# shunpeizhang/nebula

Measured on AMD Instinct MI355X. Metric: GO 3 STEPS traversed edges/sec (TEPS) at 1/2/4/8 GPU; FIND SHORTEST PATH p50, higher is better.
Workload: dtype int64; 1 GPU; GO 3 STEPS FROM <root> OVER e WHERE e.w < 50 YIELD e._dst, 16 single-root queries per step; graph=RMAT-26, parts=100, roots=16, queries_in_flight=6, parallelism=single, vertices_rank0=32799492, live_edges_out_plus_in_rank0=2120776948

## Files before the change

### nebula_amd/csrc/kernels.hip

```cpp
#include <hip/hip_runtime.h>
#include <array>
#include <cstddef>

#include <cstdio>
#include <cstring>
#include <vector>

#include "aggops.h"
#include "stage.h"
#include "ws.h"

namespace nbg {


struct DegSrc {
  const uint32_t* row_ptr;
  const uint8_t* visible;
  uint32_t cap;
};

struct ListOut {
  uint32_t* ids;
  uint32_t* seg_end;
  uint32_t* seg_rs;
// ... 2607 lines not shown
    launch(dim3(mark_grid(il->n, il->total)), 0, w->stream, a, nullptr, w->seg_end, w->seg_rs, w->flags, FinalParams{},
           bp, &w->q->e_st[step][tix], &w->q->step_n[step], il);
    prof_end(w, p, K_EXPAND_MARK, step, tix);
    return hipGetLastError();
  }
  const ListRef L = prepare_list(w, a0, n_bound, step, tix);
  ExpandArgs a = a0;
  a.frontier = L.ids;
  a.tsplit = set_split(w, L.set);
  FinalParams fp{};
  fp.err_flag = &w->q->err;
  hipEvent_t p = prof_begin(w, K_EXPAND_MARK);
  launch(dim3(mark_grid(n_bound, e_bound)), 0, w->stream, a, L.acc, set_end(w, L.set), set_rs(w, L.set), w->flags, fp,
         bp, &w->q->e_st[step][tix], L.stat_n, nullptr);
  prof_end(w, p, K_EXPAND_MARK, step, tix);
  return hipGetLastError();
}

void ws_set_wake(Workspace* w, bool flag) { w->wake_flag = flag; }

void ws_set_mark_claims(Workspace* w, bool claims) {
  const bool flags = w->env_flags || !claims;
  if (flags != w->mark_flags) (void)hipMemsetAsync(&w->q->acc[2], 0, 3 * sizeof(unsigned long long), w->stream);
  w->mark_flags = flags;
}

hipError_t ws_finish_step(Workspace* w, int step, const ExpandArgs* next0) {
  if (w->mark_flags) return ws_compact(w, step, next0);
  w->cur ^= 1;
  w->list_acc = &w->q->acc[2 + (step + 1) % 3];
  w->seg_ready = next0 != nullptr;
  return hipSuccess;
}

hipError_t ws_compact(Workspace* w, int step, const ExpandArgs* next0) {
  unsigned long long* acc = &w->q->acc[2 + w->pc];
  unsigned long long* other = &w->q->acc[2 + (w->pc ^ 1)];
  w->pc ^= 1;
  uint32_t* next = w->frontier[w->cur ^ 1];
  hipEvent_t p = prof_begin(w, K_COMPACT);
  hipLaunchKernelGGL(k_compact, dim3((unsigned)(w->flag_bytes / CP_BYTES)), dim3(CP_THREADS), 0, w->stream, w->flags,
                     deg_src(next0), list_out(w, next, acc, other, nullptr, w->cur ^ 1));
  prof_end(w, p, K_COMPACT, step, 0);
  w->cur ^= 1;
  w->list_acc = acc;
  w->seg_ready = next0 != nullptr;
  return hipGetLastError();
}

static int edge_columns_read(const TypeProgram& prog) {
  uint64_t seen = 0;
  int n = 0;
  for (auto& ins : prog.code) {
    if (ins.op != OP_COL && ins.op != OP_COLV) continue;
    const uint64_t bit = 1ull << (ins.aux & 63);
    if (!(seen & bit)) { seen |= bit; ++n; }
  }
  return n;
}

static const void* col_ptr(const ExpandArgs& a, int c, int* bytes) {
  if (a.hnarrow && a.hnarrow[c]) {
    *bytes = a.hnarrow_bytes[c];
    return a.hnarrow[c];
  }
  *bytes = 8;
  return a.hprops[c];
}

static FastProg detect_fast(const TypeProgram& prog, const ExpandArgs& a) {
  FastProg f{};
  f.enabled = 0;
  auto leaf_col = [&](const Ins& i) {
    return (i.op == OP_COL || (i.op == OP_COLV && a.valid == nullptr)) && a.hprops != nullptr;
  };
  if (prog.where_reg >= 0) {
    if (prog.where_len != 3) return f;
    const Ins &i0 = prog.code[0], &i1 = prog.code[1], &c = prog.code[2];
    static const int kOps[6] = {OP_LT_I, OP_LE_I, OP_GT_I, OP_GE_I, OP_EQ_I, OP_NE_I};
    static const int kSwap[6] = {2, 3, 0, 1, 4, 5};
    int op = -1;
    for (int k = 0; k < 6; ++k)
      if (c.op == kOps[k]) op = k;
    if (op < 0 || c.d != prog.where_reg) return f;
    const Ins* colI = nullptr;
    const Ins* constI = nullptr;
    if (leaf_col(i0) && i1.op == OP_CONST) { colI = &i0; constI = &i1; }
    else if (i0.op == OP_CONST && leaf_col(i1)) { colI = &i1; constI = &i0; }
    else return f;
    if (c.a == colI->d && c.b == constI->d) {
    } else if (c.a == constI->d && c.b == colI->d) {
      op = kSwap[op];
    } else {
      return f;
    }
    const int64_t k = constI->imm;
    f.lo = INT64_MIN;
    f.hi = INT64_MAX;
    switch (op) {
      case 0: if (k == INT64_MIN) { f.lo = 1; f.hi = 0; } else f.hi = k - 1; break;
      case 1: f.hi = k; break;
      case 2: if (k == INT64_MAX) { f.lo = 1; f.hi = 0; } else f.lo = k + 1; break;
      case 3: f.lo = k; break;
      case 4: f.lo = f.hi = k; break;
      default: f.lo = f.hi = k; f.where_neg = 1; break;
    }
    f.has_where = 1;
    f.wcol = col_ptr(a, colI->aux, &f.wbytes);
  }
  const int ny = (int)prog.yield_reg.size();
  int pc = prog.where_len;
  for (int y = 0; y < ny; ++y) {
    if (prog.yield_reg[y] < 0) { f.ykind[y] = 4; continue; }
    if (pc >= (int)prog.code.size()) return f;
    const Ins& i = prog.code[pc++];
    if (i.d != prog.yield_reg[y]) return f;
    if (i.op == OP_DST) { f.ykind[y] = 0; f.dst_yield = 1; }
    else if (i.op == OP_SRC) f.ykind[y] = 1;
    else if (i.op == OP_RANK) f.ykind[y] = 2;
    else if (i.op == OP_EIDX) f.ykind[y] = 5;
    else if (leaf_col(i)) { f.ykind[y] = 3; f.ycol[y] = col_ptr(a, i.aux, &f.ybytes[y]); }
    else return f;
  }
  if (pc != (int)prog.code.size()) return f;
  f.enabled = 1;
  return f;
}

static unsigned final_grid(uint64_t n_bound, uint64_t e_bound) {
  const char* ev = getenv("NBG_FINAL_GRID");
  const unsigned cap = ev ? (unsigned)atoi(ev) : 0u;
  const unsigned g = expand_grid(n_bound, e_bound);
  return cap && cap < g ? cap : g;
}

unsigned ws_final_grid(uint64_t n_bound, uint64_t e_bound) { return final_grid(n_bound, e_bound); }

uint64_t ws_final_blk_cap(uint64_t n_bound, uint64_t e_bound) {
  const uint64_t tiles = cdiv(n_bound + e_bound + 1, TILE);
  const uint64_t waves = (uint64_t)final_grid(n_bound, e_bound) * WAVES;
  return cdiv(tiles, waves) * WAVES * TILE;
}

uint64_t ws_shard_cap(uint64_t n_bound, uint64_t e_bound) {
  uint64_t tiles = cdiv(n_bound + e_bound + 1, TILE);
  return cdiv(tiles, NSHARD) * TILE;
}

static bool lean_final() {
  static const bool on = !getenv("NBG_FINAL_LEAN") || atoi(getenv("NBG_FINAL_LEAN")) != 0;
  return on;
}

static bool final_where_shape(const FastProg& f, const ExpandArgs& a) {
  bool dst_only = f.enabled != 0;
  for (int y = 0; y < MAX_YIELDS; ++y) dst_only = dst_only && (f.ykind[y] == 0 || f.ykind[y] == 4);
  return dst_only && lean_final() && f.dst_yield && a.dst_vid && f.has_where && f.wcol;
}

bool ws_final_where(const TypeProgram& prog, const ExpandArgs& a, StmtIndexSpec* sp) {
  if (prog.yield_reg.size() > (size_t)MAX_YIELDS) return false;
  const FastProg f = detect_fast(prog, a);
  if (!final_where_shape(f, a)) return false;
  sp->row_ptr = a.row_ptr;
  sp->dst_vid = a.dst_vid;
  sp->wcol = f.wcol;
  sp->wbytes = f.wbytes;
  sp->lo = f.lo;
  sp->hi = f.hi;
  sp->where_neg = f.where_neg;
  return true;
}

hipError_t ws_expand_final(Workspace* w, const ExpandArgs& a0, uint64_t n_bound, uint64_t e_bound, int step, int tix,
                           const TypeProgram& prog, uint64_t region_base, uint64_t blk_cap, const InlineList* il,
                           const uint32_t* full_row_ptr) {
  if (step > MAX_STEPS || tix >= MAX_TYPES_Q) return hipErrorInvalidValue;
  const bool inl = inline_start_list(w, tix, il);
  if (full_row_ptr && (inl || tix != 0 || !w->seg_ready)) return hipErrorInvalidValue;
  const ListRef L = inl ? ListRef{nullptr, nullptr, &w->q->step_n[step], 0} : prepare_list(w, a0, n_bound, step, tix);
  ExpandArgs a = a0;
  a.frontier = L.ids;
  a.tsplit = inl ? nullptr : set_split(w, L.set);
  uint32_t* const l_end = set_end(w, L.set);
  uint32_t* const l_rs = set_rs(w, L.set);
  FinalParams fp{};
  fp.prog = w->d_prog + (size_t)tix * MAX_PROGRAM;
  fp.where_len = prog.where_len;
  fp.where_reg = prog.where_reg;
  fp.prog_len = (int)prog.code.size();
  fp.nyields = (int)prog.yield_reg.size();
  for (int y = 0; y < fp.nyields; ++y) {
    fp.yield_reg[y] = prog.yield_reg[y];
    fp.yield_const[y] = prog.yield_const[y];
  }
  for (int y = 0; y < MAX_YIELDS; ++y) fp.out_cols[y] = ws_row_col(w, y < w->ncols_alloc ? y : 0);
  fp.region_base = region_base;
  fp.blk_cap = blk_cap;
  fp.blk_rows = w->blk_rows + (size_t)tix * EXPAND_GRID;
  fp.err_flag = &w->q->err;
  fp.probe_mask = prog.probe_mask;
  fp.keep_on_error = prog.keep_on_error ? 1 : 0;
  fp.tag_bits = &w->q->tagbits;
  a.str.arena = w->sarena;
  a.str.arena_cap = w->sarena_cap;
  a.str.arena_used = &w->q->arena_used;
  a.str.err_flag = &w->q->err;
  fp.fast = detect_fast(prog, a);
  if (full_row_ptr) {
    if (!final_where_shape(fp.fast, a)) return hipErrorInvalidValue;
    fp.fast.has_where = 0;
    fp.fast.wcol = nullptr;
    fp.fast.wbytes = 0;
  }
  size_t lds = fp.fast.enabled ? 0 : (size_t)(prog.nregs > 0 ? prog.nregs : 1) * BLOCK * sizeof(int64_t);
  bool dst_only = fp.fast.enabled;
  for (int y = 0; y < fp.nyields; ++y) dst_only = dst_only && (fp.fast.ykind[y] == 0 || fp.fast.ykind[y] == 4);
  const bool wide = fp.fast.enabled && !dst_only && fp.nyields >= 4 && e_bound <= (1ull << 20);
  hipEvent_t p = prof_begin(w, K_EXPAND_FINAL);
  const dim3 grid(final_grid(n_bound, e_bound));
  unsigned long long* e_st = &w->q->e_st[step][tix];
  const auto launch = dst_only ? launch_expand<FINALD>
                      : wide ? launch_expand<FINALY>
                      : fp.fast.enabled ? launch_expand<FINALF> : launch_expand<FINAL>;
  if (!inl && dst_only && lean_final() && fp.fast.dst_yield && a.dst_vid && (!fp.fast.has_where || fp.fast.wcol)) {
    FinalDstArgs fa{};
    fa.acc = L.acc;
    fa.seg_end = l_end;
    fa.seg_rs = l_rs;
    fa.tsplit = a.tsplit;
    fa.tsplit_n = w->cap_tiles;
    fa.dst_vid = a.dst_vid;
    fa.wcol = fp.fast.wcol;
    fa.lo = fp.fast.lo;
    fa.hi = fp.fast.hi;
    fa.where_neg = fp.fast.where_neg;
    fa.nyields = fp.nyields;
    for (int y = 0; y < fp.nyields; ++y) {
      if (fp.fast.ykind[y] != 0) fa.const_mask |= 1ull << y;
      fa.yconst[y] = fp.yield_const[y];
      fa.out[y] = fp.out_cols[y];
    }
    fa.region_base = region_base;
    fa.blk_cap = blk_cap;
    fa.blk_rows = fp.blk_rows;
    fa.stat_e = e_st;
    if (full_row_ptr) {
      fa.full_rp = full_row_ptr;
      fa.ids = L.ids;
      fa.visible = a.visible;
    }
    fa.stat_n = L.stat_n;
    fa.err_flag = &w->q->err;
    const bool one = fp.nyields == 1 && fa.const_mask == 0;
    const hipError_t le = launch_final_dst(fa, fp.fast.has_where ? fp.fast.wbytes : 0, one, grid.x, w->stream);
    if (le != hipSuccess) {
      prof_end(w, p, K_EXPAND_FINAL, step, tix, 0.0, 0.0);
      return le;
    }
  } else {
    launch(grid, lds, w->stream, a, L.acc, l_end, l_rs, w->flags, fp, BfsParams{}, e_st, L.stat_n, inl ? il : nullptr);
  }
  prof_end(w, p, K_EXPAND_FINAL, step, tix, full_row_ptr ? -1.0 : (double)edge_columns_read(prog), (double)fp.nyields);
  w->final_grid[tix] = final_grid(n_bound, e_bound);
  return hipGetLastError();
}



hipError_t ws_backtracker(Workspace* w, int64_t** out, int64_t** in) {
  if (!w->bt) HIP_TRY(hipMalloc((void**)&w->bt, (w->nv + 1) * 8));
  if (w->comm && !w->h_btc) {
    const uint64_t G = (uint64_t)w->comm->world, nwords = G * w->npad / 64;
    if (!w->bt_out) HIP_TRY(hipMalloc((void**)&w->bt_out, G * w->npad * 8));
    if (!w->bt_pack) HIP_TRY(hipMalloc((void**)&w->bt_pack, G * w->npad * 8));
    if (!w->bt_recv) HIP_TRY(hipMalloc((void**)&w->bt_recv, G * w->npad * 8));
    if (!w->bt_pre) HIP_TRY(hipMalloc((void**)&w->bt_pre, 2 * nwords * 4));
    if (!w->bt_boff) HIP_TRY(hipMalloc((void**)&w->bt_boff, 2 * (nwords / RW_BLOCK) * 4));
    if (!w->bt_disp) HIP_TRY(hipMalloc((void**)&w->bt_disp, 2 * G * 8));
    HIP_TRY(hipHostMalloc((void**)&w->h_btc, 2 * G * 8, hipHostMallocMapped | hipHostMallocCoherent));
    HIP_TRY(hipHostGetDevicePointer((void**)&w->d_btc, w->h_btc, 0));
  }
  w->bt_active = true;
  *in = w->bt;
  *out = w->comm ? w->bt_out : w->bt;
  return hipSuccess;
}

void ws_backtracker_off(Workspace* w) { w->bt_active = false; }

hipError_t ws_scan_only(Workspace* w, const ExpandArgs& a, uint64_t n_bound, int step, int tix) {
  const ListRef L = prepare_list(w, a, n_bound, step, tix);
  hipLaunchKernelGGL(k_note, dim3(1), dim3(1), 0, w->stream, L.acc, &w->q->e_st[step][tix], L.stat_n);
  return hipGetLastError();
}




struct Wake {
  unsigned long long* word;
  unsigned int* ticket;
  unsigned long long seq;
};
__device__ void wake_host(const Wake& wk) {
  if (!wk.word) return;
  __builtin_amdgcn_fence(__ATOMIC_RELEASE, "");
  __syncthreads();
  if (threadIdx.x != 0) return;
  if (gridDim.x > 1) {
    const unsigned got = __hip_atomic_fetch_add(wk.ticket, 1u, __ATOMIC_RELEASE, __HIP_MEMORY_SCOPE_AGENT);
    if (got != gridDim.x - 1) return;
    __builtin_amdgcn_fence(__ATOMIC_ACQUIRE, "agent");
    __hip_atomic_store(wk.ticket, 0u, __ATOMIC_RELAXED, __HIP_MEMORY_SCOPE_AGENT);
  }
  __hip_atomic_store(wk.word, wk.seq, __ATOMIC_RELEASE, __HIP_MEMORY_SCOPE_SYSTEM);
}

__global__ void __launch_bounds__(BLOCK) k_q_out(unsigned long long* __restrict__ src, unsigned long long* dst,
                                                 uint32_t n8, uint32_t nq8, Wake wk) {
  for (uint32_t i = threadIdx.x; i < n8; i += BLOCK) {
    dst[i] = src[i];
    if (i < nq8) src[i] = 0;
  }
  wake_host(wk);
}

static bool wake_by_flag() {
  static const bool on = !(getenv("NBG_WAKE") && strcmp(getenv("NBG_WAKE"), "event") == 0) &&
                         getenv("NBG_BLOCKING_SYNC") == nullptr;
  return on;
}

static Wake arm_wake(Workspace* w) {
  w->wake_armed = wake_by_flag() && w->wake_flag && !w->comm;
  if (!w->wake_armed) return Wake{nullptr, nullptr, 0};
  return Wake{w->d_wake, w->d_ticket, ++w->wake_seq};
}

static hipError_t wait_wake(Workspace* w) {
  const unsigned long long want = w->wake_seq;
  for (unsigned k = 1;; ++k) {
    if (__atomic_load_n(w->h_wake, __ATOMIC_ACQUIRE) == want) {
      (void)hipEventQuery(w->done_ev);
      return hipSuccess;
    }
    if ((k & 255) == 0) {
      const hipError_t e = hipEventQuery(w->done_ev);
      if (e == hipErrorNotReady) continue;
      if (__atomic_load_n(w->h_wake, __ATOMIC_ACQUIRE) == want) return hipSuccess;
      return e == hipSuccess ? hipErrorLaunchFailure : e;
    }
  }
}

hipError_t ws_end_query_async(Workspace* w) {
  int nt = 0;
  for (int t = 0; t < MAX_TYPES_Q; ++t)
    if (w->final_grid[t]) nt = t + 1;
  static_assert(sizeof(QState) % 8 == 0 && EXPAND_GRID % 2 == 0, "k_q_out copies 8-byte words");
  const size_t bytes = sizeof(QState) + (size_t)nt * EXPAND_GRID * 4;
  const Wake wk = arm_wake(w);
  hipLaunchKernelGGL(k_q_out, dim3(1), dim3(BLOCK), 0, w->stream, reinterpret_cast<unsigned long long*>(w->q),
                     reinterpret_cast<unsigned long long*>(w->d_hq), (uint32_t)(bytes / 8),
                     (uint32_t)(sizeof(QState) / 8), wk);
  w->q_reset = true;
  HIP_TRY(hipGetLastError());
  if (w->h_small) w->h_small[0] = 0;
  if (!w->done_ev) HIP_TRY(hipEventCreateWithFlags(&w->done_ev, hipEventDisableTiming));
  return hipEventRecord(w->done_ev, w->stream);
}

hipError_t ws_end_query_wait(Workspace* w) {
  static const bool blocking = getenv("NBG_BLOCKING_SYNC") != nullptr;
  if (w->comm) {
    HIP_TRY(ws_sync(w));
  } else if (w->wake_armed) {
    w->wake_armed = false;
    HIP_TRY(wait_wake(w));
  } else if (blocking) {
    HIP_TRY(hipEventSynchronize(w->done_ev));
  } else {
    hipError_t e;
    while ((e = hipEventQuery(w->done_ev)) == hipErrorNotReady) {
    }
    HIP_TRY(e);
  }
  if (!w->q_reset) HIP_TRY(hipMemsetAsync(w->q, 0, sizeof(QState), w->stream));
  w->q_reset = false;
  prof_flush(w, w->h_q);
  return hipSuccess;
}

constexpr int SMALL_SEGS = 2048;
constexpr int SMALL_WGS = 16;
__global__ void __launch_bounds__(BLOCK) k_q_out_small(unsigned long long* __restrict__ src, unsigned long long* dst,
                                                       uint32_t n8, uint32_t nq8, const uint32_t* __restrict__ blk_rows, SmallPack sp,
                                                       int64_t* const* __restrict__ cols, int64_t* small, Wake wk) {
  for (uint32_t i = blockIdx.x * BLOCK + threadIdx.x; i < n8; i += gridDim.x * BLOCK) {
    dst[i] = src[i];
    if (i < nq8) src[i] = 0;
  }
  __shared__ uint32_t s_seg[SMALL_SEGS];
  __shared__ uint32_t s_off[SMALL_SEGS + 1];
  __shared__ uint32_t s_lds[WAVES];
  __shared__ uint32_t s_n, s_rows;
  if (threadIdx.x == 0) s_n = s_rows = 0;
  __syncthreads();
// ... 1453 lines not shown
```

### nebula_amd/csrc/nbg_internal.h

```cpp
#pragma once
#include <hip/hip_runtime_api.h>

#include <array>
#include <cstdint>
#include <map>
#include <memory>
#include <string>
#include <unordered_map>
#include <vector>

#include "../../include/nbg.h"

namespace nbg {

constexpr uint32_t NO_ROW = 0xFFFFFFFFu;

struct Column {
  std::string name;
  int32_t type;
};
struct Schema {
  int64_t version = 0;
  std::vector<Column> cols;
  int find(const std::string& n) const {
// ... 166 lines not shown
constexpr uint64_t STR_HASH_MASK = ((uint64_t)1 << 62) - 1;
inline bool is_derived_code(int64_t c) { return ((uint64_t)c >> 62) == 1; }
constexpr int64_t STR_INPUT = (int64_t)1 << 61;
constexpr int64_t STR_ARENA = (int64_t)1 << 60;
inline bool is_input_code(int64_t c) { return ((uint64_t)c >> 61) == 1; }
constexpr uint64_t STR_HASH_INIT = 0xcbf29ce484222325ull;

#if defined(__HIPCC__)
#define NBG_HD __host__ __device__
#else
#define NBG_HD
#endif
NBG_HD inline uint64_t str_hash_step(uint64_t h, uint8_t b) { return (h ^ b) * 0x100000001b3ull; }
NBG_HD inline int64_t str_derived_code(uint64_t h, uint64_t len) {
  uint64_t z = h ^ (len * 0x9E3779B97F4A7C15ull);
  z = (z ^ (z >> 30)) * 0xBF58476D1CE4E5B9ull;
  z = (z ^ (z >> 27)) * 0x94D049BB133111EBull;
  z ^= z >> 31;
  return STR_DERIVED | (int64_t)(z & STR_HASH_MASK);
}

struct DevStrings {
  const uint32_t* off = nullptr;
  const char* bytes = nullptr;
  const int64_t* s2i = nullptr;
  const int64_t* s2f = nullptr;
  const uint8_t* s2ok = nullptr;
  uint64_t n = 0;
  const uint32_t* xoff = nullptr;
  const char* xbytes = nullptr;
  uint64_t xn = 0;
  char* arena = nullptr;
  unsigned long long* arena_used = nullptr;
  uint64_t arena_cap = 0;
  unsigned long long* err_flag = nullptr;
};
constexpr unsigned long long ARENA_OVERFLOW = 1ull << 32;
constexpr unsigned long long SPLIT_BAD = 1ull << 48;

constexpr int MAX_REGS = 48;
int interp_max_regs();
int tiny_max_regs();
constexpr int MAX_PROGRAM = 256;
constexpr int MAX_YIELDS = 32;

struct TypeProgram {
  int32_t etype = 0;
  std::vector<Ins> code;
  int where_len = 0;
  int where_reg = -1;
  VKind where_kind = VK_BOOL;
  bool where_const = false;
  bool where_const_val = true;
  bool where_always_error = false;
  std::vector<int> yield_reg;
  std::vector<VKind> yield_kind;
  std::vector<int64_t> yield_const;
  std::vector<std::string> yield_const_str;
  std::vector<Ins> data;
  bool sout = false;
  uint64_t sout_bytes = 0;
  bool needs_error_check = false;
  uint32_t probe_mask = 0;
  bool keep_on_error = false;
  int nregs = 0;
};

#ifndef NBG_VT
#define NBG_VT 4
#endif
constexpr int VT = NBG_VT;
constexpr int TILE = 64 * VT;
constexpr int NSHARD = 64;
constexpr int MAX_STEPS = 32;
constexpr int MAX_TYPES_Q = 32;
constexpr int INLINE_STARTS = 32;
constexpr int MAX_TAG_BITS = 16;
constexpr int MAX_INPUT_COLS = 32;

struct InlineList {
  uint32_t n;
  uint32_t n_in;
  uint32_t total;
  uint32_t id[INLINE_STARTS];
  uint32_t end[INLINE_STARTS];
  uint32_t rs[INLINE_STARTS];
};

struct QState {
  unsigned long long n;
  unsigned long long total;
  unsigned long long err;
  unsigned long long acc[5];
  unsigned long long step_n[MAX_STEPS + 2];
  unsigned long long e_st[MAX_STEPS + 2][MAX_TYPES_Q];
  unsigned long long tagbits;
  unsigned long long arena_used;
};

struct ExpandArgs {
  const uint32_t* frontier;
  const uint32_t* row_ptr;
  const uint32_t* col;
  const int64_t* dst_vid;
  const int64_t* rank;
  const uint8_t* valid;
  const uint8_t* visible;
  const int64_t* vids;
  const int64_t* const* props;
  uint32_t cap;
  const uint32_t* tsplit;
  const int64_t* const* hprops;
  void* const* hnarrow;
  const int* hnarrow_bytes;
  const int64_t* const* tcols;
  const uint8_t* const* tpres;
  uint32_t gbase;
  int64_t* bt;
  const int64_t* bt_in;
  int bt_first;
  const int64_t* in_ids;
  uint64_t in_n;
  const int64_t* const* in_cols;
  DevStrings str;
  int64_t now_sec;
  uint64_t rand_seed;
};

struct FinalDstArgs {
  const unsigned long long* acc;
  const uint32_t* seg_end;
  const uint32_t* seg_rs;
  const uint32_t* tsplit;
  uint64_t tsplit_n;
  const int64_t* dst_vid;
  const void* wcol;
  int64_t lo, hi;
  int32_t where_neg;
  int32_t nyields;
  uint64_t const_mask;
  int64_t yconst[MAX_YIELDS];
  int64_t* out[MAX_YIELDS];
  uint64_t region_base, blk_cap;
  uint32_t* blk_rows;
  unsigned long long* stat_e;
  unsigned long long* stat_n;
  unsigned long long* err_flag;
  const uint32_t* full_rp;
  const uint32_t* ids;
  const uint8_t* visible;
};
hipError_t launch_final_dst(const FinalDstArgs& a, int wbytes, bool one, unsigned grid, hipStream_t s);

struct StmtIndexSpec {
  const uint32_t* row_ptr;
  const int64_t* dst_vid;
  uint64_t nv, edges;
  const void* wcol;
  int wbytes;
  int64_t lo, hi;
  int where_neg;
};
struct StmtIndex {
  uint32_t* rp = nullptr;
  int64_t* dst = nullptr;
  uint64_t rows = 0;
  uint64_t bytes = 0;
};
bool stmtidx_build(const StmtIndexSpec& sp, uint64_t budget_bytes, hipStream_t s, StmtIndex* out, double* ms);
void stmtidx_free(StmtIndex* ix);

constexpr int LVL_BITS = 6;
constexpr uint32_t MAX_PATH_LEN = (1u << LVL_BITS) - 1;
constexpr int PSLOTS = 8;
enum PathLabel { LAB_F = 0, LAB_B = 1, LAB_S = 2, LAB_M = 3, NUM_LABS = 4 };
constexpr int GREEDY_HOP_BLOCKS = 64;
constexpr int PATH_REC = 64;

struct PState {
  unsigned long long n[PSLOTS];
  unsigned long long total;
  unsigned long long edges;
  unsigned long long meets;
  unsigned long long found;
  unsigned long long err;
  unsigned long long acc[2];
  unsigned long long dsum[2];
  unsigned long long shard[NSHARD];
  unsigned long long ln[PATH_REC];
  unsigned long long le[PATH_REC];
  unsigned long long lc[PATH_REC];
  unsigned long long gticket;
  unsigned long long gv;
  unsigned long long gpart[4 * GREEDY_HOP_BLOCKS];
  unsigned long long ld[PATH_REC];
  unsigned long long mdsum;
  unsigned long long mdsum_out;
};

struct PathTypes {
  int n = 0;
  int32_t type[MAX_TYPES_Q];
  ExpandArgs a[MAX_TYPES_Q];
};

struct SpTypes {
  int n = 0;
  int32_t type[MAX_TYPES_Q];
  const uint32_t* row_ptr[MAX_TYPES_Q];
  const uint32_t* col[MAX_TYPES_Q];
  const int64_t* dst_vid[MAX_TYPES_Q];
  const int64_t* rank[MAX_TYPES_Q];
  uint64_t ne[MAX_TYPES_Q];
};
struct SpResult {
  unsigned long long L;
  unsigned long long edges;
  unsigned long long err;
  unsigned long long levels;
  unsigned long long abytes;
  unsigned long long launches;
  unsigned long long batches;
  long long path[1 + 3 * MAX_PATH_LEN];
};
constexpr unsigned long long CH_ERR_WALK_CAP = 64;
inline std::string sp_err_text(unsigned long long err) {
  if (err == CH_ERR_WALK_CAP) return "greedy walk incomplete at the chain's launch cap";
  if (err & 4) return "a frontier list's merge-path split did not describe its tile (code " + std::to_string(err) + ")";
  return "device search aborted (code " + std::to_string(err) + ")";
}
constexpr uint32_t CH_LAB_WORDS = 4;
struct SpCtx;
enum SpMode : int { SP_CHAIN = 1 };
SpCtx* sp_create(uint64_t nv, uint64_t item_cap, uint64_t edge_cap, hipStream_t s, std::string* err);
void sp_destroy(SpCtx* c);
hipError_t sp_launch(SpCtx* c, const SpTypes& fwd, const SpTypes& bwd, const uint8_t* visible, const int64_t* vids,
                     uint32_t s, uint32_t t, uint32_t upto, uint64_t dmin = 0);
bool sp_ready(SpCtx* c);
struct SpPair {
  const SpTypes* fwd;
  const SpTypes* bwd;
  const uint8_t* visible;
  const int64_t* vids;
  uint32_t s, t, upto;
};
hipError_t sp_launch_batch(SpCtx* const* cs, int n, const SpPair* pairs);
struct ChainCtx;
ChainCtx* chain_create(uint64_t nv, uint64_t edge_cap, hipStream_t s, std::string* err, uint64_t list_cap = 0);
void sp_set_list_cap(SpCtx* c, uint64_t list_cap);
void chain_destroy(ChainCtx* c);
hipError_t chain_launch(ChainCtx* c, const SpTypes& fwd, const SpTypes& bwd, const uint8_t* visible,
                        const int64_t* vids, uint32_t* const lab[3], uint32_t epoch, uint32_t s, uint32_t t,
                        uint32_t upto, uint64_t dmin = 0);
bool chain_more(ChainCtx* c, hipError_t* he);
bool chain_woken(const ChainCtx* c);
struct ChainQuery {
  const SpTypes* fwd;
  const SpTypes* bwd;
  const uint8_t* visible;
  const int64_t* vids;
  uint32_t* const* lab;
  uint32_t epoch, s, t, upto;
};
hipError_t chain_launch_batch(ChainCtx* const* cs, int n, const ChainQuery* qs);
struct ChainSlot {
  ChainCtx* c;
  uint32_t* const* lab;
  uint32_t ebase;
};
constexpr uint32_t CH_ROLL_UPTO = 32;
constexpr int CH_ROLL_SLOTS = 64;
hipError_t chain_roll(const ChainSlot* slots, int nslots, const SpTypes& fwd, const SpTypes& bwd,
                      const uint8_t* visible, const int64_t* vids, const uint32_t* s, const uint32_t* t, uint32_t n,
                      uint32_t upto, SpResult* results);
hipError_t sp_roll(SpCtx* const* cs, int nslots, const SpTypes& fwd, const SpTypes& bwd, const uint8_t* visible,
                   const int64_t* vids, const uint32_t* s, const uint32_t* t, uint32_t n, uint32_t upto,
                   SpResult* results);
void chain_result(const ChainCtx* c, SpResult* out);
constexpr int CHAIN_KINDS = 4;
extern const char* const kChainKernelNames[CHAIN_KINDS];
void chain_profile(ChainCtx* c, int mode);
void chain_profile_done(ChainCtx* c, const SpResult& r);
void chain_profile_accum(const ChainCtx* c, double* launches, double* ms, double* bytes);
void sp_profile(SpCtx* c, int mode);
hipError_t sp_reserve_chain(SpCtx* c);
void sp_profile_accum(const SpCtx* c, double* launches, double* ms, double* bytes);
hipError_t sp_wait(SpCtx* c, SpResult* out);

struct Comm {
  int world = 1, rank = 0;
  std::string last;
  virtual ~Comm();
  virtual const char* kind() const = 0;
  int agree(hipStream_t s, int32_t local, int32_t* out);
  int gather_u64(hipStream_t s, const uint64_t* mine, size_t k, std::vector<uint64_t>* out);
  virtual void abort() { aborted = true; }
  bool is_aborted() const { return aborted; }
  int wait(hipStream_t s);
  virtual int alltoall(const void* send, void* recv, size_t bytes, hipStream_t s) = 0;
  virtual int alltoallv(const void* send, const uint64_t* scount, const uint64_t* sdisp, void* recv,
                        const uint64_t* rcount, const uint64_t* rdisp, size_t elem, hipStream_t s) = 0;
  virtual int allgather(const void* send, void* recv, size_t bytes, hipStream_t s) = 0;
  virtual int allreduce_sum_u64(unsigned long long* buf, size_t n, hipStream_t s) = 0;
  virtual Comm* split(std::string* err) {
    (void)err;
    return nullptr;
// ... 491 lines not shown
```

Baseline: 546.1 billion TEPS.

## Add dedicated final-step copy kernel for pre-filtered dst-only index path

Adds a specialised kernel for the last GO step when a prebuilt statement index (full_row_ptr) already holds filtered destination ids and only one dst yield is needed. Each wave handles 512-row output chunks. It finds the owning segment through a pipelined multi-level ballot search over seg_end, copies contiguous runs with 16-byte vector loads, and uses nontemporal stores. Chunks that span segment boundaries are resolved through an LDS bitmask and delta table. This is meant to replace the more general final_dst kernel's per-edge work with streaming copies, at the cost of added complexity and a SPLIT_BAD fallback flag if a chunk has too many segments.

```diff
diff --git a/nebula_amd/csrc/finalcopy.hip b/nebula_amd/csrc/finalcopy.hip
--- /dev/null
+++ b/nebula_amd/csrc/finalcopy.hip
@@ -0,0 +1,251 @@
+#include <hip/hip_runtime.h>
+
+#include "nbg_internal.h"
+
+namespace nbg {
+namespace {
+
+constexpr int CB = 256;
+constexpr int CW = CB / 64;
+constexpr int CH = 512;
+constexpr int CM = CH / 64;
+constexpr int CI = CH / 128;
+static_assert(CH % 128 == 0, "a chunk is whole 16-byte stores of 64 lanes");
+
+typedef long long row2 __attribute__((ext_vector_type(2), aligned(8)));
+
+__device__ __forceinline__ void wave_lds_sync() {
+  __builtin_amdgcn_fence(__ATOMIC_RELEASE, "wavefront");
+  __builtin_amdgcn_wave_barrier();
+  __builtin_amdgcn_fence(__ATOMIC_ACQUIRE, "wavefront");
+}
+
+template <typename T>
+__device__ __forceinline__ T ld(const T* p) {
+  return __hip_atomic_load(p, __ATOMIC_RELAXED, __HIP_MEMORY_SCOPE_WAVEFRONT);
+}
+
+__device__ __forceinline__ uint32_t lanes_below(unsigned long long b) {
+  return __builtin_amdgcn_mbcnt_hi((uint32_t)(b >> 32), __builtin_amdgcn_mbcnt_lo((uint32_t)b, 0u));
+}
+
+}
+
+__global__ void __launch_bounds__(CB) __attribute__((amdgpu_waves_per_eu(8)))
+k_final_copy(FinalCopyArgs a) {
+  __shared__ unsigned long long sMaskAll[CW][CM];
+  __shared__ uint32_t sDeltaAll[CW][CH + 1];
+  const int lane = threadIdx.x & 63;
+  const int w = __builtin_amdgcn_readfirstlane(threadIdx.x >> 6);
+  unsigned long long* const sMask = sMaskAll[w];
+  uint32_t* const sDelta = sDeltaAll[w];
+  const uint32_t g = gridDim.x * CW;
+  const uint32_t t_first = blockIdx.x * CW + w;
+  const unsigned long long packed = *a.acc;
+  const uint64_t n = packed >> 32;
+  const uint32_t n32 = (uint32_t)n, total = (uint32_t)packed;
+  if (blockIdx.x == 0 && threadIdx.x == 0) {
+    if (a.stat_e && !a.full_rp) *a.stat_e += total;
+    if (a.stat_n) *a.stat_n = n;
+  }
+  const uint32_t nfull = total / CH;
+  const uint32_t nlast = n32 ? n32 - 1 : 0u;
+  int64_t* const out = a.out + a.region_base;
+  const uint32_t step1 = (n32 + 63) / 64;
+  const uint32_t probe1 = ld(a.seg_end + ((uint32_t)(lane + 1) * step1 - 1 < nlast ? (uint32_t)(lane + 1) * step1 - 1 : nlast));
+  auto probe = [&](uint32_t lo, uint32_t hi, uint32_t step) -> uint32_t {
+    const uint32_t at = lo + (uint32_t)(lane + 1) * step - 1;
+    return ld(a.seg_end + (at < hi - 1 ? at : hi - 1));
+  };
+  auto narrow = [&](uint32_t* lo, uint32_t* hi, uint32_t step, uint32_t v, uint32_t r) {
+    *lo += (uint32_t)__popcll(__ballot(v <= r)) * step;
+    if (*lo >= *hi) *lo = *hi - 1;
+    *hi = *hi - *lo < step ? *hi : *lo + step;
+  };
+  auto begin = [&](uint32_t r, uint32_t* lo, uint32_t* hi) {
+    *lo = 0;
+    *hi = n32;
+    if (n32 > 64) narrow(lo, hi, step1, probe1, r);
+    while (*hi - *lo > 64u * 64u * 64u) {
+      const uint32_t step = (*hi - *lo + 63) / 64;
+      narrow(lo, hi, step, probe(*lo, *hi, step), r);
+    }
+  };
+  auto bracket = [&](uint32_t r) -> uint32_t {
+    uint32_t lo, hi;
+    begin(r, &lo, &hi);
+    while (hi - lo > 64) {
+      const uint32_t step = (hi - lo + 63) / 64;
+      narrow(&lo, &hi, step, probe(lo, hi, step), r);
+    }
+    return lo;
+  };
+  auto stage = [&](uint32_t s0, uint32_t* x0, uint32_t* x1, uint32_t* rr) {
+    const uint32_t q = s0 + (uint32_t)lane;
+    const uint32_t c0 = q == 0 ? 0u : (q - 1 < n32 ? q - 1 : nlast);
+    const uint32_t c1 = q < n32 ? q : nlast;
+    *x0 = ld(a.seg_end + c0);
+    *x1 = ld(a.seg_end + c1);
+    *rr = ld(a.seg_rs + c1);
+  };
+  auto window = [&](uint32_t s0, uint32_t x0, uint32_t x1, uint32_t rr, uint32_t* st, uint32_t* en, uint32_t* r) {
+    const uint32_t q = s0 + (uint32_t)lane;
+    *st = q == 0 ? 0u : (q - 1 < n32 ? x0 : 0xFFFFFFFFu);
+    *en = q < n32 ? x1 : 0xFFFFFFFFu;
+    *r = q < n32 ? rr : 0u;
+  };
+  auto resolve = [&](uint32_t kb, uint32_t r0, uint32_t nb, uint32_t st, uint32_t en, uint32_t rs,
+                     uint32_t (&idx)[2 * CI]) -> bool {
+    const uint32_t r1 = r0 + nb;
+    if (lane < CM) sMask[lane] = 0;
+    uint32_t heads = 0;
+    bool first_ok = false, reached = false;
+    for (uint32_t s0 = kb;; s0 += 64) {
+      if (s0 != kb) {
+        uint32_t x0, x1, rr;
+        stage(s0, &x0, &x1, &rr);
+        window(s0, x0, x1, rr, &st, &en, &rs);
+      }
+      const bool in = s0 + (uint32_t)lane < n32;
+      const uint32_t lo = st > r0 ? st : r0, hi = en < r1 ? en : r1;
+      const bool head = in && lo < hi;
+      const unsigned long long hb = __ballot(head);
+      const uint32_t rank = heads + 1 + lanes_below(hb);
+      if (head && rank <= (uint32_t)CH) {
+        const uint32_t p = lo - r0;
+        sDelta[rank] = rs - st;
+        atomicOr(&sMask[p >> 6], 1ull << (p & 63));
+      }
+      if (heads == 0 && hb) first_ok = __ballot(head && lo == r0) != 0;
+      heads += (uint32_t)__popcll(hb);
+      reached = __ballot(in && en >= r1) != 0;
+      if (reached || nlast - s0 < 64) break;
+    }
+    wave_lds_sync();
+    const bool ok = first_ok && reached && heads <= (uint32_t)CH;
+    uint32_t before = 0;
+    const int hw = lane >> 5;
+    const int b0 = (2 * lane) & 63;
+    const unsigned long long le0 = ~0ull >> (63 - b0), le1 = ~0ull >> (62 - b0);
+#pragma unroll
+    for (int i = 0; i < CI; ++i) {
+      const unsigned long long m0 = sMask[2 * i], m1 = sMask[2 * i + 1];
+      const uint32_t c0 = (uint32_t)__popcll(m0);
+      const unsigned long long m = hw ? m1 : m0;
+      const uint32_t base = before + (hw ? c0 : 0u);
+      const uint32_t p = (uint32_t)(i * 128 + 2 * lane);
+      idx[2 * i] = r0 + p + sDelta[base + (uint32_t)__popcll(m & le0)];
+      idx[2 * i + 1] = r0 + p + 1 + sDelta[base + (uint32_t)__popcll(m & le1)];
+      before += c0 + (uint32_t)__popcll(m1);
+    }
+    wave_lds_sync();
+    const uint32_t jsafe = ok ? (uint32_t)__builtin_amdgcn_readfirstlane((int)idx[0]) : 0u;
+#pragma unroll
+    for (int i = 0; i < CI; ++i) {
+      const uint32_t p = (uint32_t)(i * 128 + 2 * lane);
+      if (!ok || p >= nb) idx[2 * i] = jsafe;
+      if (!ok || p + 1 >= nb) idx[2 * i + 1] = jsafe;
+    }
+    return ok;
+  };
+  auto store2 = [&](int64_t* p, row2 v) { __builtin_nontemporal_store(v, reinterpret_cast<row2*>(p)); };
+  auto store_chunk = [&](const row2 (&v)[CI], uint32_t tt) {
+    int64_t* const o = out + (uint64_t)tt * CH + 2 * lane;
+#pragma unroll
+    for (int i = 0; i < CI; ++i) store2(o + i * 128, v[i]);
+  };
+  auto fetch = [&](uint32_t tt, uint32_t kb, uint32_t x0, uint32_t x1, uint32_t rr, row2 (&v)[CI]) {
+    const uint32_t r0 = tt * CH;
+    uint32_t st, en, rs;
+    window(kb, x0, x1, rr, &st, &en, &rs);
+    const unsigned long long own = __ballot(kb + (uint32_t)lane < n32 && st <= r0 && r0 < en);
+    const int l0 = own ? __ffsll((long long)own) - 1 : 0;
+    const uint32_t st0 = (uint32_t)__builtin_amdgcn_readlane((int)st, l0);
+    const uint32_t en0 = (uint32_t)__builtin_amdgcn_readlane((int)en, l0);
+    const uint32_t rs0 = (uint32_t)__builtin_amdgcn_readlane((int)rs, l0);
+    if (own && en0 - r0 >= (uint32_t)CH) {
+      const int64_t* const src = a.dst_vid + (uint64_t)(rs0 + (r0 - st0)) + 2 * lane;
+#pragma unroll
+      for (int i = 0; i < CI; ++i) v[i] = *reinterpret_cast<const row2*>(src + i * 128);
+    } else {
+      uint32_t idx[2 * CI];
+      const bool ok = resolve(kb, r0, CH, st, en, rs, idx);
+      if (!ok && lane == 0) atomicOr(a.err_flag, SPLIT_BAD);
+#pragma unroll
+      for (int i = 0; i < CI; ++i) {
+        v[i].x = ld(a.dst_vid + idx[2 * i]);
+        v[i].y = ld(a.dst_vid + idx[2 * i + 1]);
+      }
+    }
+  };
+  const uint32_t mine = t_first < nfull ? (nfull - 1 - t_first) / g + 1 : 0u;
+  uint32_t a_lo = 0, a_hi = 0, a_step = 0, a_val = 0, b_lo = 0, b_hi = 0, b_step = 0, b_val = 0;
+  bool a_pend = false, b_pend = false;
+  uint32_t s_kb = 0, s_x0 = 0, s_x1 = 0, s_rr = 0;
+  row2 cur[CI];
+#pragma unroll
+  for (int i = 0; i < CI; ++i) cur[i] = row2{0, 0};
+  for (uint32_t it = 0; mine && it < mine + 4; ++it) {
+    if (it >= 4) store_chunk(cur, t_first + (it - 4) * g);
+    if (it >= 3 && it < mine + 3) fetch(t_first + (it - 3) * g, s_kb, s_x0, s_x1, s_rr, cur);
+    if (it >= 2 && it < mine + 2) {
+      if (b_pend) narrow(&b_lo, &b_hi, b_step, b_val, (t_first + (it - 2) * g) * CH);
+      s_kb = b_lo;
+      stage(s_kb, &s_x0, &s_x1, &s_rr);
+    }
+    if (it >= 1 && it < mine + 1) {
+      b_lo = a_lo;
+      b_hi = a_hi;
+      if (a_pend) narrow(&b_lo, &b_hi, a_step, a_val, (t_first + (it - 1) * g) * CH);
+      b_pend = b_hi - b_lo > 64;
+      if (b_pend) {
+        b_step = (b_hi - b_lo + 63) / 64;
+        b_val = probe(b_lo, b_hi, b_step);
+      }
+    }
+    if (it < mine) {
+      begin((t_first + it * g) * CH, &a_lo, &a_hi);
+      a_pend = a_hi - a_lo > 64;
+      if (a_pend) {
+        a_step = (a_hi - a_lo + 63) / 64;
+        a_val = probe(a_lo, a_hi, a_step);
+      }
+    }
+  }
+  const uint32_t rem = total - nfull * CH;
+  if (rem && t_first == nfull % g) {
+    const uint32_t r0 = nfull * CH;
+    const uint32_t kb = bracket(r0);
+    uint32_t x0, x1, rr, st, en, rs, idx[2 * CI];
+    stage(kb, &x0, &x1, &rr);
+    window(kb, x0, x1, rr, &st, &en, &rs);
+    const bool ok = resolve(kb, r0, rem, st, en, rs, idx);
+    if (!ok && lane == 0) atomicOr(a.err_flag, SPLIT_BAD);
+    int64_t v[2 * CI];
+#pragma unroll
+    for (int i = 0; i < 2 * CI; ++i) v[i] = ld(a.dst_vid + idx[i]);
+#pragma unroll
+    for (int i = 0; i < CI; ++i) {
+      const uint32_t p = (uint32_t)(i * 128 + 2 * lane);
+      if (ok && p < rem) out[(uint64_t)r0 + p] = v[2 * i];
+      if (ok && p + 1 < rem) out[(uint64_t)r0 + p + 1] = v[2 * i + 1];
+    }
+  }
+  if (a.full_rp) {
+    unsigned long long sum = 0;
+    for (uint64_t i = (uint64_t)t_first * 64 + lane; i < n; i += (uint64_t)g * 64) {
+      const uint32_t v = a.ids[i];
+      if (v != NO_ROW && (!a.visible || a.visible[v])) sum += a.full_rp[v + 1] - a.full_rp[v];
+    }
+    for (int o = 32; o; o >>= 1) sum += __shfl_down(sum, o, 64);
+    if (lane == 0 && sum) atomicAdd(a.stat_e, sum);
+  }
+  if (threadIdx.x == 0) a.blk_rows[blockIdx.x] = blockIdx.x == 0 ? total : 0u;
+}
+
+hipError_t launch_final_copy(const FinalCopyArgs& a, unsigned grid, hipStream_t s) {
+  hipLaunchKernelGGL(k_final_copy, dim3(grid), dim3(CB), 0, s, a);
+  return hipGetLastError();
+}
+
+}
diff --git a/nebula_amd/csrc/kernels.hip b/nebula_amd/csrc/kernels.hip
--- a/nebula_amd/csrc/kernels.hip
+++ b/nebula_amd/csrc/kernels.hip
@@ -2783,6 +2783,11 @@
   return on;
 }
 
+static bool final_copy_on() {
+  const char* ev = getenv("NBG_FINAL_COPY");
+  return !ev || atoi(ev) != 0;
+}
+
 static bool final_where_shape(const FastProg& f, const ExpandArgs& a) {
   bool dst_only = f.enabled != 0;
   for (int y = 0; y < MAX_YIELDS; ++y) dst_only = dst_only && (f.ykind[y] == 0 || f.ykind[y] == 4);
@@ -2884,7 +2889,26 @@
     fa.stat_n = L.stat_n;
     fa.err_flag = &w->q->err;
     const bool one = fp.nyields == 1 && fa.const_mask == 0;
-    const hipError_t le = launch_final_dst(fa, fp.fast.has_where ? fp.fast.wbytes : 0, one, grid.x, w->stream);
+    hipError_t le;
+    if (full_row_ptr && one && final_copy_on()) {
+      FinalCopyArgs ca{};
+      ca.acc = fa.acc;
+      ca.seg_end = fa.seg_end;
+      ca.seg_rs = fa.seg_rs;
+      ca.dst_vid = fa.dst_vid;
+      ca.out = fa.out[0];
+      ca.region_base = region_base;
+      ca.blk_rows = fa.blk_rows;
+      ca.stat_e = fa.stat_e;
+      ca.stat_n = fa.stat_n;
+      ca.err_flag = fa.err_flag;
+      ca.full_rp = fa.full_rp;
+      ca.ids = fa.ids;
+      ca.visible = fa.visible;
+      le = launch_final_copy(ca, grid.x, w->stream);
+    } else {
+      le = launch_final_dst(fa, fp.fast.has_where ? fp.fast.wbytes : 0, one, grid.x, w->stream);
+    }
     if (le != hipSuccess) {
       prof_end(w, p, K_EXPAND_FINAL, step, tix, 0.0, 0.0);
       return le;
diff --git a/nebula_amd/csrc/nbg_internal.h b/nebula_amd/csrc/nbg_internal.h
--- a/nebula_amd/csrc/nbg_internal.h
+++ b/nebula_amd/csrc/nbg_internal.h
@@ -342,6 +342,23 @@
 };
 hipError_t launch_final_dst(const FinalDstArgs& a, int wbytes, bool one, unsigned grid, hipStream_t s);
 
+struct FinalCopyArgs {
+  const unsigned long long* acc;
+  const uint32_t* seg_end;
+  const uint32_t* seg_rs;
+  const int64_t* dst_vid;
+  int64_t* out;
+  uint64_t region_base;
+  uint32_t* blk_rows;
+  unsigned long long* stat_e;
+  unsigned long long* stat_n;
+  unsigned long long* err_flag;
+  const uint32_t* full_rp;
+  const uint32_t* ids;
+  const uint8_t* visible;
+};
+hipError_t launch_final_copy(const FinalCopyArgs& a, unsigned grid, hipStream_t s);
+
 struct StmtIndexSpec {
   const uint32_t* row_ptr;
   const int64_t* dst_vid;
```

Measured after the change: 571.8 billion TEPS (median of 6 runs). 1.05x the previous value.
